# THUDM/GCC

Measured on NVIDIA H100. Metric: subgraphs/sec (MoCo pretrain step), higher is better.
Workload: dtype f32

## Files before the change

gcc_b200/csrc/sampler.cu:

```cuda
#include "common.cuh"

namespace gccb {

__global__ void draw_seeds_kernel(const double* __restrict__ cdf, int64_t n, uint64_t key,
                                  int64_t first, int count, int64_t* __restrict__ seeds,
                                  int64_t* __restrict__ sample_ids) {
  int i = blockIdx.x * blockDim.x + threadIdx.x;
  if (i >= count) return;
  uint64_t sample = (uint64_t)(first + i);
  u32x4 w = philox_at(key, sample, 0, 0, 0, GCCB_TAG_SEED);
  uint64_t u53 = ((uint64_t)w.x << 21) | (uint64_t)(w.y >> 11);
  double u = (double)u53 * (1.0 / 9007199254740992.0);
  int64_t lo = 0, hi = n;
  while (lo < hi) {
    int64_t mid = (lo + hi) >> 1;
    if (cdf[mid] > u) hi = mid; else lo = mid + 1;
  }
  seeds[i] = lo < n ? lo : n - 1;
  if (sample_ids) sample_ids[i] = first + i;
}

__device__ __forceinline__ int local_id(const int* keys, int n, int seed, int u) {
  if (u == seed) return 0;
  int lo = 1, hi = n;
// ... 3 lines not shown
  }
  return (lo < n && keys[lo] == u) ? lo : -1;
}

__device__ __forceinline__ unsigned bloom_bit(int u) { return ((unsigned)u * 2654435761u) >> 16; }

__device__ __forceinline__ int adj_count(const int32_t* __restrict__ indices, int64_t beg, int64_t end, int u) {
  const int64_t stop = end;
  while (beg < end) {
    int64_t mid = (beg + end) >> 1;
    if (indices[mid] < u) beg = mid + 1; else end = mid;
  }
  if (beg >= stop || indices[beg] != u) return 0;
  const int32_t* run = indices + beg;
  int lo = 1, hi = (int)min(stop - beg, (int64_t)0x7fffffff);
  if (lo == hi || run[lo] != u) return 1;
  while (lo < hi) {
    int mid = (lo + hi) >> 1;
    if (run[mid] <= u) lo = mid + 1; else hi = mid;
  }
  return lo;
}
#define GCCB_REVERSE_FACTOR 16
#ifndef GCCB_ST
#define GCCB_ST 1024
#endif
#define GCCB_SW (GCCB_ST / 32)
#ifndef GCCB_SCAN_UNROLL
#define GCCB_SCAN_UNROLL 4
#endif
#ifndef GCCB_BLOOM
#define GCCB_BLOOM 1
#endif
#define GCCB_BLOOM_WORDS 2048
#ifndef GCCB_HUB_LIST
#define GCCB_HUB_LIST 1024
#endif
#define GCCB_HIT_STAGE 128
#ifndef GCCB_WALK_KEYS
#define GCCB_WALK_KEYS 32768
#endif
#define GCCB_WALK_BUDGET_MAX (GCCB_WALK_KEYS - (int)GCCB_HOPCAP)
#define GCCB_WIDE_CTAS 32
#define GCCB_WIDE_KEYS_MAX (1 << 30)

__device__ void block_sort_pad(int* a, int cnt) {
  const int tid = threadIdx.x;
  int P = 1;
  while (P < cnt) P <<= 1;
  for (int i = cnt + tid; i < P; i += GCCB_ST) a[i] = 0x7fffffff;
  __syncthreads();
  for (int k = 2; k <= P; k <<= 1) {
    for (int j = k >> 1; j > 0; j >>= 1) {
      for (int i = tid; i < P; i += GCCB_ST) {
        const int ixj = i ^ j;
        if (ixj > i) {
          const int x = a[i], y = a[ixj];
          if ((x > y) == ((i & k) == 0)) { a[i] = y; a[ixj] = x; }
        }
      }
      __syncthreads();
    }
  }
}

__device__ __forceinline__ bool in_sorted(const int* a, int n, int u) {
  int lo = 0, hi = n;
  while (lo < hi) { const int mid = (lo + hi) >> 1; if (a[mid] < u) lo = mid + 1; else hi = mid; }
  return lo < n && a[lo] == u;
}

__device__ int ns_expand(const int64_t* __restrict__ indptr, const int32_t* __restrict__ indices, uint64_t key,
                         uint64_t sample, uint32_t view, int seed, int hops, int k, int cap, int* V, int* F, int* S,
                         int* scan_scratch, int32_t* __restrict__ subv, int* layers) {
  __shared__ int s_miss;
  const int tid = threadIdx.x, lane = tid & 31, warp = tid >> 5;
  int nV = 1, nF = 1, checked = 0, hop = 1;
// ... 7 lines not shown
      int64_t beg = 0, d = 0;
      if (i < nF) { beg = indptr[F[i]]; d = indptr[F[i] + 1] - beg; }
      int tot;
      const int ex = block_scan_excl(d <= k ? (int)d : k, scan_scratch, &tot);
      if (i < nF) {
        int* out = S + nc + ex;
        if (d <= k) {
          for (int e = 0; e < (int)d; ++e) out[e] = indices[beg + e];
        } else {
          for (int t = 0; t < k; ++t) {
            const uint32_t j = (uint32_t)(d - k + t);
            const u32x4 w = philox_at(key, sample, (uint32_t)i | ((uint32_t)t << 16), c3hop, view, c3tag);
            const int r = (int)__umulhi(w.x, j + 1u);
            bool dup = false;
            for (int q = 0; q < t; ++q) dup |= out[q] == r;
            out[t] = dup ? (int)j : r;
          }
          for (int t = 0; t < k; ++t) out[t] = indices[beg + out[t]];
        }
      }
      nc += tot;
    }
    __syncthreads();
    block_sort_pad(S, nc);
    int nF2 = 0;
    for (int b0 = 0; b0 < nc; b0 += GCCB_ST) {
      const int i = b0 + tid;
      const int head = i < nc && (i == 0 || S[i - 1] != S[i]);
      int tot;
      const int ex = block_scan_excl(head, scan_scratch, &tot);
      if (head && nF2 + ex < cap) F[nF2 + ex] = S[i];
      nF2 += tot;
    }
    if (nF2 > cap) return -1;
    nF = nF2;
    __syncthreads();
    if (nF == 0) break;
    int nNew = 0;
    for (int b0 = 0; b0 < nF; b0 += GCCB_ST) {
      const int i = b0 + tid;
      const int fresh = i < nF && !in_sorted(V, nV, F[i]);
      int tot;
      const int ex = block_scan_excl(fresh, scan_scratch, &tot);
      if (fresh) S[nV + nNew + ex] = F[i];
      nNew += tot;
    }
    if (nV + nNew > cap) return -1;
    if (nNew > 0) {
      for (int i = tid; i < nV; i += GCCB_ST) S[i] = V[i];
      block_sort_pad(S, nV + nNew);
      nV += nNew;
      for (int i = tid; i < nV; i += GCCB_ST) V[i] = S[i];
      __syncthreads();
    } else if (nV != checked) {
      if (tid == 0) s_miss = 0;
      __syncthreads();
      int miss = 0;
      for (int i = warp; i < nV; i += GCCB_SW) {
        const int64_t end = indptr[V[i] + 1];
        for (int64_t e = indptr[V[i]] + lane; e < end && !miss; e += 32) miss = !in_sorted(V, nV, indices[e]);
      }
      if (miss) s_miss = 1;
      __syncthreads();
      const bool closed = s_miss == 0;
      __syncthreads();
      if (closed) break;
      checked = nV;
    }
  }
  *layers = hop > hops ? hops : hop;
  for (int i = tid; i < nV; i += GCCB_ST) {
    const int v = V[i];
    subv[v < seed ? i + 1 : (v == seed ? 0 : i)] = v;
  }
  return nV;
}

__device__ __forceinline__ int rwr_node_set(const int64_t* __restrict__ indptr, const int32_t* __restrict__ indices,
                                            int budget, uint32_t restart_thresh, uint64_t key, uint64_t sample,
                                            int view, int64_t seed64, int seed, int* keys, int* scan_scratch,
                                            int* s_tstar, int* s_m, int32_t* __restrict__ flags,
                                            int32_t* rest, int* steps) {
  const int tid = threadIdx.x;
  if (tid == 0) *s_tstar = 0x7fffffff;
  __syncthreads();

  int base = 0;
  int total = 0;
  for (int chunk = 0;; ++chunk) {
    const uint32_t t = (uint32_t)(chunk * GCCB_ST + tid);
    int len = 1;
    for (uint32_t hop = 1; hop < GCCB_HOPCAP; ++hop) {
      u32x4 w = philox_at(key, sample, t, hop, (uint32_t)view, GCCB_TAG_WALK);
      if (w.x < restart_thresh) break;
      ++len;
    }
    int chunk_total;
    int excl = block_scan_excl(len, scan_scratch, &chunk_total);
    int cum = base + excl + len;
    if (cum >= budget && cum - len < budget) *s_tstar = (int)t;
    __syncthreads();
    const int tstar = *s_tstar;
    if ((int)t <= tstar) {
      int64_t cur = seed64;
      int pos = base + excl;
      for (uint32_t hop = 0; hop < (uint32_t)len; ++hop) {
        u32x4 w = philox_at(key, sample, t, hop, (uint32_t)view, GCCB_TAG_WALK);
        int64_t beg = indptr[cur];
        uint32_t deg = (uint32_t)(indptr[cur + 1] - beg);
        if (deg == 0u) { atomicOr(flags, (int)GCCB_FLAG_ZERO_DEGREE); keys[pos++] = (int)cur; continue; }
        cur = indices[beg + __umulhi(w.y, deg)];
        keys[pos++] = (int)cur;
      }
    }
    if (tstar != 0x7fffffff) {
      if ((int)t == tstar) *s_m = cum;
      __syncthreads();
      total = *s_m;
      break;
    }
    base += chunk_total;
    __syncthreads();
  }
  __syncthreads();
  if (tid == 0) *s_m = 0;

  int P = 1;
  while (P < total) P <<= 1;
  for (int i = total + tid; i < P; i += GCCB_ST) keys[i] = 0x7fffffff;
  __syncthreads();
  for (int k = 2; k <= P; k <<= 1) {
    for (int j = k >> 1; j > 0; j >>= 1) {
      for (int i = tid; i < P; i += GCCB_ST) {
        int ixj = i ^ j;
        if (ixj > i) {
          int a = keys[i], b = keys[ixj];
          bool asc = (i & k) == 0;
          if ((a > b) == asc) { keys[i] = b; keys[ixj] = a; }
        }
      }
      __syncthreads();
    }
  }
  int n_rest = 0;
  for (int b0 = 0; b0 < total; b0 += GCCB_ST) {
    int i = b0 + tid;
    int head = 0, v = 0;
    if (i < total) {
      v = keys[i];
      head = (v != seed) && (i == 0 || keys[i - 1] != v);
    }
    int cnt;
    int ex = block_scan_excl(head, scan_scratch, &cnt);
    if (head) rest[n_rest + ex] = v;
    n_rest += cnt;
  }
  *steps = total;
  return n_rest + 1;
}

enum { kModeRwr = 0, kModePairs = 1, kModeNs = 2 };

struct WideWs {
  int32_t* subv;
  int32_t* subdeg;
  int32_t* rowstart;
  unsigned long long* used;
  unsigned* next;
  int region;
};

template <int kMode, bool kWide>
__device__ __forceinline__ void
walk_slot(const int slot, int* keys, const int64_t* __restrict__ indptr, const int32_t* __restrict__ indices,
          int64_t n_nodes, const int32_t* __restrict__ budget_table, int budget_table_len, uint32_t restart_thresh,
          uint64_t key, const int64_t* __restrict__ seeds, const int64_t* __restrict__ sample_ids, int B, int cap_n,
          int32_t* __restrict__ subv_scratch, int32_t* __restrict__ subdeg_scratch,
          int32_t* __restrict__ rowstart_scratch, int32_t* __restrict__ pool, int pool_cap,
          unsigned long long* __restrict__ pool_counter, int64_t* __restrict__ counters,
          int32_t* __restrict__ flags, const int64_t* __restrict__ seeds_k, int ns_hops, int ns_k, int node_cap,
          const WideWs& wide) {
  __shared__ int scan_scratch[33];
  __shared__ int stage[GCCB_SW][GCCB_HIT_STAGE];
  __shared__ int s_tstar, s_m;
  __shared__ unsigned long long s_sumdeg;
  __shared__ int s_nhub, s_pos;
  __shared__ unsigned bloom[GCCB_BLOOM_WORDS];
  __shared__ int hub_rows[GCCB_HUB_LIST];
  const int tid = threadIdx.x, lane = tid & 31, warp = tid >> 5;
  const int view = slot / B, g = slot - view * B;
  int64_t seed64 = seeds[g];
  seed64 = seed64 < 0 ? 0 : (seed64 >= n_nodes ? n_nodes - 1 : seed64);
  const int64_t q64 = seed64;
  if constexpr (kMode != kModeRwr) {
    if (view == 1) {
      seed64 = seeds_k[g];
      seed64 = seed64 < 0 ? 0 : (seed64 >= n_nodes ? n_nodes - 1 : seed64);
    }
  }
  const int seed = (int)seed64;
  const uint64_t sample = (uint64_t)sample_ids[g];
  int32_t* subv = subv_scratch + (size_t)slot * cap_n;
  int32_t* subdeg = subdeg_scratch + (size_t)slot * cap_n;
  int32_t* rowstart = rowstart_scratch + (size_t)slot * cap_n;
  if (tid == 0) { s_m = 0; s_sumdeg = 0ull; }
  int n, total = 0;
  if constexpr (kMode == kModeNs) {
    n = ns_expand(indptr, indices, key, sample, (uint32_t)view, seed, ns_hops, ns_k, cap_n, keys, keys + cap_n,
                  keys + 2 * cap_n, scan_scratch, subv, &total);
    if (n < 0) {
      if (tid == 0) {
        counters[(size_t)slot * 4 + 0] = (int64_t)node_cap + 1;
        counters[(size_t)slot * 4 + 1] = 0;
        counters[(size_t)slot * 4 + 2] = total;
        counters[(size_t)slot * 4 + 3] = 0;
        atomicOr(flags, (int)GCCB_FLAG_NODE_OVERFLOW);
      }
      return;
    }
    __syncthreads();
  } else {
    const int64_t sdeg = indptr[q64 + 1] - indptr[q64];
    const int budget = budget_table[sdeg < budget_table_len ? (int)sdeg : budget_table_len - 1];
    if constexpr (!kWide) {
      if (budget > GCCB_WALK_BUDGET_MAX) {
        if (tid == 0) subv[0] = -1;
        return;
      }
    }
    n = rwr_node_set(indptr, indices, budget, restart_thresh, key, sample, view, seed64, seed, keys, scan_scratch,
                     &s_tstar, &s_m, flags, kWide ? keys : subv + 1, &total);
  }
  if constexpr (kWide) {
    if (tid == 0) {
      const unsigned long long off = atomicAdd(wide.used + view, (unsigned long long)n);
      s_pos = off + (unsigned long long)n <= (unsigned long long)wide.region ? (int)off : -1;
      subv[1] = s_pos;
    }
    __syncthreads();
    const int off = s_pos;
    if (off < 0) {
      if (tid == 0) {
        counters[(size_t)slot * 4 + 0] = n;
        counters[(size_t)slot * 4 + 1] = n - 1;
        counters[(size_t)slot * 4 + 2] = total;
        counters[(size_t)slot * 4 + 3] = 0;
      }
      return;
    }
    const size_t at = (size_t)view * wide.region + off;
    subv = wide.subv + at;
    subdeg = wide.subdeg + at;
    rowstart = wide.rowstart + at;
    for (int i = tid; i < n - 1; i += GCCB_ST) subv[1 + i] = keys[i];
    if (tid == 0) subv[0] = seed;
    keys = subv;
  } else {
    if (tid == 0) subv[0] = seed;
    __syncthreads();
    for (int i = tid; i < n; i += GCCB_ST) keys[i] = subv[i];
  }
  for (int i = tid; i < GCCB_BLOOM_WORDS; i += GCCB_ST) bloom[i] = 0u;
  __syncthreads();
  for (int i = tid; i < n; i += GCCB_ST) {
    const unsigned b = bloom_bit(keys[i]);
    atomicOr(&bloom[b >> 5], 1u << (b & 31u));
  }
  __syncthreads();

  int* wstage = stage[warp];
  const unsigned lt_mask = (1u << lane) - 1u;
  int m_local = 0;
  unsigned long long sumdeg_local = 0ull;
  int sr = 0;
  {
    int lo = 1, hi = n;
    while (lo < hi) { int mid = (lo + hi) >> 1; if (keys[mid] < seed) lo = mid + 1; else hi = mid; }
    sr = lo - 1;
  }
  if (tid == 0) s_nhub = 0;
  __syncthreads();
  for (int i = tid; i < n; i += GCCB_ST) {
    const int64_t v = keys[i];
    int mark = -3;
    if (indptr[v + 1] - indptr[v] > (int64_t)GCCB_REVERSE_FACTOR * n) {
      const int idx = atomicAdd(&s_nhub, 1);
      if (idx < GCCB_HUB_LIST) { hub_rows[idx] = i; mark = -2; }
    }
    rowstart[i] = mark;
  }
  __syncthreads();
  const int n_hub = min(s_nhub, GCCB_HUB_LIST);
  for (int h = 0; h < n_hub; ++h) {
    const int i = hub_rows[h];
    const int64_t v = keys[i];
    const int64_t beg = indptr[v], end = indptr[v + 1];
    int cnt = 0, my_j = 0, my_c = 0, my_ex = 0;
    for (int t0 = 0; t0 < n; t0 += GCCB_ST) {
      const int t = t0 + tid;
      int j = 0, c = 0;
      if (t < n) {
        j = t < sr ? t + 1 : (t == sr ? 0 : t);
        c = adj_count(indices, beg, end, keys[j]);
      }
      int tot;
      const int ex = block_scan_excl(c, scan_scratch, &tot);
      if (t0 == 0) { my_j = j; my_c = c; my_ex = ex; }
      cnt += tot;
    }
    if (tid == 0) {
      const unsigned long long p64 = cnt > 0 ? atomicAdd(pool_counter, (unsigned long long)cnt) : 0ull;
      s_pos = p64 + (unsigned long long)cnt > (unsigned long long)pool_cap ? -1 : (int)p64;
    }
    __syncthreads();
    const int pos = s_pos;
    if (pos >= 0) {
      if (n <= GCCB_ST) {
        for (int k = 0; k < my_c; ++k) pool[pos + my_ex + k] = my_j;
      } else {
        int w = 0;
        for (int t0 = 0; t0 < n; t0 += GCCB_ST) {
          const int t = t0 + tid;
          int j = 0, c = 0;
          if (t < n) {
            j = t < sr ? t + 1 : (t == sr ? 0 : t);
            c = adj_count(indices, beg, end, keys[j]);
          }
          int tot;
          const int ex = block_scan_excl(c, scan_scratch, &tot);
          for (int k = 0; k < c; ++k) pool[pos + w + ex + k] = j;
          w += tot;
        }
      }
    }
    if (tid == 0) {
      subdeg[i] = cnt;
      rowstart[i] = pos;
      m_local += cnt;
      sumdeg_local += (unsigned long long)(end - beg);
    }
    __syncthreads();
  }
  for (int i = warp; i < n; i += GCCB_SW) {
    if (rowstart[i] != -3) continue;
    const int64_t v = keys[i];
    const int64_t beg = indptr[v], end = indptr[v + 1];
    const bool reverse = end - beg > (int64_t)GCCB_REVERSE_FACTOR * n;
    int pos = 0, w = 0, round = 0;
    auto emit = [&](int j) {
      const unsigned hit = __ballot_sync(0xffffffffu, j >= 0);
      if (j >= 0) {
        const int q = w + __popc(hit & lt_mask);
        if (round == 1) pool[pos + q] = j;
        else if (q < GCCB_HIT_STAGE) wstage[q] = j;
      }
      w += __popc(hit);
    };
    auto scan_row = [&]() {
      w = 0;
      if (reverse) {
        for (int t0 = 0; t0 < n; t0 += 32) {
          const int t = t0 + lane;
          int j = 0, c = 0;
          if (t < n) {
            j = t < sr ? t + 1 : (t == sr ? 0 : t);
            c = adj_count(indices, beg, end, keys[j]);
// ... 47 lines not shown
    }
    __syncwarp();
    if (lane == 0) {
      subdeg[i] = cnt;
      rowstart[i] = pos;
      m_local += cnt;
      sumdeg_local += (unsigned long long)(end - beg);
    }
  }
  if (lane == 0) {
    atomicAdd(&s_m, m_local);
    atomicAdd(&s_sumdeg, sumdeg_local);
  }
  __syncthreads();
  if (tid == 0) {
    counters[(size_t)slot * 4 + 0] = n;
    counters[(size_t)slot * 4 + 1] = s_m;
    counters[(size_t)slot * 4 + 2] = total;
    counters[(size_t)slot * 4 + 3] = (int64_t)s_sumdeg;
  }
}

template <int kMode>
__global__ void __launch_bounds__(GCCB_ST)
rwr_walk_unique_kernel(const int64_t* __restrict__ indptr, const int32_t* __restrict__ indices, int64_t n_nodes,
                       const int32_t* __restrict__ budget_table, int budget_table_len,
                       uint32_t restart_thresh, uint64_t key, const int64_t* __restrict__ seeds,
                       const int64_t* __restrict__ sample_ids, int B, int cap_n,
                       int32_t* __restrict__ subv_scratch, int32_t* __restrict__ subdeg_scratch,
                       int32_t* __restrict__ rowstart_scratch, int32_t* __restrict__ pool, int pool_cap,
                       unsigned long long* __restrict__ pool_counter,
                       int64_t* __restrict__ counters, int32_t* __restrict__ flags,
                       const int64_t* __restrict__ seeds_k, int ns_hops, int ns_k, int node_cap) {
  GCCB_DYN_SMEM(int, keys);
  walk_slot<kMode, false>(blockIdx.x, keys, indptr, indices, n_nodes, budget_table, budget_table_len, restart_thresh,
                          key, seeds, sample_ids, B, cap_n, subv_scratch, subdeg_scratch, rowstart_scratch, pool,
                          pool_cap, pool_counter, counters, flags, seeds_k, ns_hops, ns_k, node_cap, WideWs{});
}

template <int kMode>
__global__ void __launch_bounds__(GCCB_ST)
rwr_walk_wide_kernel(const int64_t* __restrict__ indptr, const int32_t* __restrict__ indices, int64_t n_nodes,
                     const int32_t* __restrict__ budget_table, int budget_table_len,
                     uint32_t restart_thresh, uint64_t key, const int64_t* __restrict__ seeds,
                     const int64_t* __restrict__ sample_ids, int B, int cap_n,
                     int32_t* __restrict__ subv_scratch, int32_t* __restrict__ pool, int pool_cap,
                     unsigned long long* __restrict__ pool_counter,
                     int64_t* __restrict__ counters, int32_t* __restrict__ flags,
                     const int64_t* __restrict__ seeds_k, WideWs wide, int32_t* __restrict__ wide_keys,
                     size_t keys_len) {
  __shared__ int s_slot;
  int* keys = wide_keys + (size_t)blockIdx.x * keys_len;
  for (;;) {
    if (threadIdx.x == 0) s_slot = (int)atomicAdd(wide.next, 1u);
    __syncthreads();
    const int slot = s_slot;
    if (slot >= 2 * B) return;
    if (subv_scratch[(size_t)slot * cap_n] < 0)
      walk_slot<kMode, true>(slot, keys, indptr, indices, n_nodes, budget_table, budget_table_len, restart_thresh,
                             key, seeds, sample_ids, B, cap_n, subv_scratch, nullptr, nullptr, pool, pool_cap,
                             pool_counter, counters, flags, seeds_k, 0, 0, 0, wide);
    __syncthreads();
  }
}

__global__ void __launch_bounds__(256)
batch_offsets_kernel(const int64_t* __restrict__ counters, int B, int node_cap, int edge_cap,
                     int32_t* __restrict__ node_off, int32_t* __restrict__ edge_off,
                     int32_t* __restrict__ flags) {
  __shared__ int scan_scratch[33];
  const int view = blockIdx.x, tid = threadIdx.x;
  long long nbase = 0, ebase = 0;
  for (int b0 = 0; b0 < B; b0 += 256) {
    int g = b0 + tid;
    int n = 0, m = 0;
    if (g < B) {
      n = (int)counters[(size_t)(view * B + g) * 4 + 0];
      m = (int)counters[(size_t)(view * B + g) * 4 + 1];
    }
    int tn, tm;
    int en = block_scan_excl(n, scan_scratch, &tn);
    int em = block_scan_excl(m, scan_scratch, &tm);
    if (g < B) {
      long long no = nbase + en, eo = ebase + em;
      node_off[view * (B + 1) + g] = (int)(no > 0x7fffffffLL ? 0x7fffffffLL : no);
      edge_off[view * (B + 1) + g] = (int)(eo > 0x7fffffffLL ? 0x7fffffffLL : eo);
    }
    nbase += tn;
    ebase += tm;
  }
  if (tid == 0) {
    int f = 0;
    if (nbase > node_cap) { f |= GCCB_FLAG_NODE_OVERFLOW; }
    if (ebase > edge_cap) { f |= GCCB_FLAG_EDGE_OVERFLOW; }
    node_off[view * (B + 1) + B] = f ? -1 : (int)nbase;
    edge_off[view * (B + 1) + B] = f ? -1 : (int)ebase;
    if (f) atomicOr(flags, f);
  }
}

template <bool kWide>
__device__ __forceinline__ void
fill_slot(const int slot, int* keys, const int64_t* __restrict__ indptr, const int32_t* __restrict__ indices,
          const int64_t* __restrict__ counters, int B, int node_cap, int edge_cap, const int32_t* __restrict__ subv,
          const int32_t* __restrict__ subdeg, const int32_t* __restrict__ rowstart, const int32_t* __restrict__ pool,
          int32_t* __restrict__ node_off, const int32_t* __restrict__ edge_off, int32_t* __restrict__ out_indptr,
          int32_t* __restrict__ out_indices, int32_t* __restrict__ out_subdeg, int32_t* __restrict__ out_graph_id,
          int32_t* __restrict__ out_orig_id) {
  __shared__ int scan_scratch[33];
  const int tid = threadIdx.x, lane = tid & 31, warp = tid >> 5;
  const int view = slot / B, g = slot - view * B;
  const int Nv = node_off[view * (B + 1) + B];
  if (Nv < 0) return;
  const int n = (int)counters[(size_t)slot * 4 + 0];
  const int noff = node_off[view * (B + 1) + g];
  const int eoff = edge_off[view * (B + 1) + g];
  int32_t* v_indptr = out_indptr + (size_t)view * (node_cap + 1);
  int32_t* v_indices = out_indices + (size_t)view * edge_cap;
  const size_t nb = (size_t)view * node_cap;
  if constexpr (!kWide)
    for (int i = tid; i < n; i += GCCB_ST) keys[i] = subv[i];
  const int seed = subv[0];
  int run = 0;
  for (int b0 = 0; b0 < n; b0 += GCCB_ST) {
    int i = b0 + tid;
    int d = i < n ? subdeg[i] : 0;
    int tot;
    int ex = block_scan_excl(d, scan_scratch, &tot);
    if (i < n) {
      v_indptr[noff + i] = eoff + run + ex;
      out_subdeg[nb + noff + i] = d;
      out_graph_id[nb + noff + i] = g;
      out_orig_id[nb + noff + i] = subv[i];
    }
    run += tot;
  }
  if (g == B - 1 && tid == 0) v_indptr[noff + n] = eoff + run;
  __syncthreads();
  for (int i = warp; i < n; i += GCCB_SW) {
    int wpos = v_indptr[noff + i];
    const int rs = rowstart[i];
    if (rs >= 0) {
      const int d = subdeg[i];
      for (int q = lane; q < d; q += 32) v_indices[wpos + q] = noff + pool[rs + q];
      continue;
    }
    const int64_t v = keys[i];
    const int64_t beg = indptr[v], end = indptr[v + 1];
    if (end - beg > (int64_t)GCCB_REVERSE_FACTOR * n) {
      int lo = 1, hi = n;
      while (lo < hi) { int mid = (lo + hi) >> 1; if (keys[mid] < seed) lo = mid + 1; else hi = mid; }
      const int sr = lo - 1;
      for (int t0 = 0; t0 < n; t0 += 32) {
        const int t = t0 + lane;
        int j = 0, c = 0;
        if (t < n) {
          j = t < sr ? t + 1 : (t == sr ? 0 : t);
          c = adj_count(indices, beg, end, keys[j]);
        }
        const int incl = warp_scan_incl(c, lane);
        for (int q = wpos + incl - c; q < wpos + incl; ++q) v_indices[q] = noff + j;
        wpos += __shfl_sync(0xffffffffu, incl, 31);
      }
      continue;
    }
    for (int64_t e0 = beg; e0 < end; e0 += 32) {
      int64_t e = e0 + lane;
      int j = -1;
      if (e < end) j = local_id(keys, n, seed, indices[e]);
      unsigned hit = __ballot_sync(0xffffffffu, j >= 0);
      if (j >= 0) v_indices[wpos + __popc(hit & ((1u << lane) - 1u))] = noff + j;
      wpos += __popc(hit);
    }
  }
}

__global__ void __launch_bounds__(GCCB_ST)
induce_fill_kernel(const int64_t* __restrict__ indptr, const int32_t* __restrict__ indices,
                   const int64_t* __restrict__ counters, int B, int cap_n, int node_cap,
                   int edge_cap, const int32_t* __restrict__ subv_scratch,
                   const int32_t* __restrict__ subdeg_scratch, const int32_t* __restrict__ rowstart_scratch,
                   const int32_t* __restrict__ pool,
                   int32_t* __restrict__ node_off, const int32_t* __restrict__ edge_off,
                   int32_t* __restrict__ out_indptr, int32_t* __restrict__ out_indices,
                   int32_t* __restrict__ out_subdeg, int32_t* __restrict__ out_graph_id,
                   int32_t* __restrict__ out_orig_id) {
  GCCB_DYN_SMEM(int, keys);
  const int slot = blockIdx.x;
  const size_t at = (size_t)slot * cap_n;
  if (subv_scratch[at] < 0) return;
  fill_slot<false>(slot, keys, indptr, indices, counters, B, node_cap, edge_cap, subv_scratch + at,
                   subdeg_scratch + at, rowstart_scratch + at, pool, node_off, edge_off, out_indptr, out_indices,
                   out_subdeg, out_graph_id, out_orig_id);
}

__global__ void __launch_bounds__(GCCB_ST)
induce_fill_wide_kernel(const int64_t* __restrict__ indptr, const int32_t* __restrict__ indices,
                        const int64_t* __restrict__ counters, int B, int cap_n, int node_cap, int edge_cap,
                        const int32_t* __restrict__ subv_scratch, WideWs wide, const int32_t* __restrict__ pool,
                        int32_t* __restrict__ node_off, const int32_t* __restrict__ edge_off,
                        int32_t* __restrict__ out_indptr, int32_t* __restrict__ out_indices,
                        int32_t* __restrict__ out_subdeg, int32_t* __restrict__ out_graph_id,
                        int32_t* __restrict__ out_orig_id) {
  const int slot = blockIdx.x;
  const int32_t* mark = subv_scratch + (size_t)slot * cap_n;
  if (mark[0] >= 0 || mark[1] < 0) return;
  const size_t at = (size_t)(slot / B) * wide.region + mark[1];
  fill_slot<true>(slot, wide.subv + at, indptr, indices, counters, B, node_cap, edge_cap, wide.subv + at,
                  wide.subdeg + at, wide.rowstart + at, pool, node_off, edge_off, out_indptr, out_indices,
                  out_subdeg, out_graph_id, out_orig_id);
}

__global__ void pair_seeds_kernel(const int64_t* __restrict__ indptr, const int32_t* __restrict__ indices,
                                  int64_t n_nodes, uint64_t key, double cdf0, double cdf1, int n_steps,
                                  const int64_t* __restrict__ seeds_q, const int64_t* __restrict__ sample_ids,
                                  int count, int64_t* __restrict__ seeds_k) {
  const int i = blockIdx.x * blockDim.x + threadIdx.x;
  if (i >= count) return;
  const uint64_t sample = (uint64_t)sample_ids[i];
  const u32x4 w = philox_at(key, sample, 0, 0, 0, GCCB_TAG_STEP);
  const double u = (double)(((uint64_t)w.x << 21) | (uint64_t)(w.y >> 11)) * (1.0 / 9007199254740992.0);
  int step = 0;
  if (step < n_steps - 1 && !(cdf0 > u)) ++step;
  if (step == 1 && step < n_steps - 1 && !(cdf1 > u)) ++step;
  int64_t cur = seeds_q[i];
  cur = cur < 0 ? 0 : (cur >= n_nodes ? n_nodes - 1 : cur);
  for (int h = 1; h <= step; ++h) {
    const int64_t beg = indptr[cur];
    const uint32_t deg = (uint32_t)(indptr[cur + 1] - beg);
    if (deg == 0u) break;
    const u32x4 r = philox_at(key, sample, 0, (uint32_t)h, 0, GCCB_TAG_KHOP);
// ... 8 lines not shown

static int pow2_ge(int x) { int p = 1; while (p < x) p <<= 1; return p; }

extern "C" int gccb_draw_seeds(const double* cdf, int64_t n_nodes, uint64_t key,
                               int64_t first_sample, int32_t count, int64_t* seeds_out,
                               int64_t* sample_ids_out, gccb_stream_t stream) {
  if (!cdf || !seeds_out || n_nodes <= 0 || count < 0) {
    set_last_error("gccb_draw_seeds: bad argument");
    return GCCB_ERR_BADARG;
  }
  if (count == 0) return GCCB_OK;
  GCCB_LAUNCH(draw_seeds_kernel, (count + 127) / 128, 128, 0, stream, cdf, n_nodes, key,
              first_sample, count, seeds_out, sample_ids_out);
  return check_launch("draw_seeds_kernel");
}

static int sampler_cap_n(int max_budget) { return (max_budget + (int)GCCB_HOPCAP + 1 + 3) & ~3; }
static bool sampler_wide(int max_budget) { return max_budget > GCCB_WALK_BUDGET_MAX; }
static int wide_region(int batch, int edge_cap) {
  const long long r = (long long)edge_cap + batch;
  return (int)(r < 0x7fffffffll ? r : 0x7fffffffll);
}
static int wide_ctas(int batch) { return 2 * batch < GCCB_WIDE_CTAS ? 2 * batch : GCCB_WIDE_CTAS; }
static size_t wide_keys_len(int max_budget) {
  size_t p = 1;
  while (p < (size_t)max_budget + GCCB_HOPCAP) p <<= 1;
  return p;
}

extern "C" size_t gccb_sample_batch_workspace(int32_t batch, int32_t max_budget, int32_t edge_cap) {
  const bool wide = sampler_wide(max_budget);
  const int cap_n = sampler_cap_n(wide ? GCCB_WALK_BUDGET_MAX : max_budget);
  size_t ints = (size_t)3 * (size_t)(2 * batch) * (size_t)cap_n + 16 + (size_t)2 * (size_t)edge_cap;
  if (wide)
    ints += (size_t)6 * (size_t)wide_region(batch, edge_cap) + (size_t)wide_ctas(batch) * wide_keys_len(max_budget);
  return ints * sizeof(int32_t);
}

template <int kMode>
static int sample_batch_rwr(const char* what, const gccb_graph_t* graph, const int64_t* seeds, const int64_t* seeds_k,
                            const int64_t* sample_ids, const gccb_batch_t* batch, void* workspace,
                            size_t workspace_bytes, gccb_stream_t stream) {
  const int B = batch->batch;
  const bool wide = sampler_wide(graph->max_budget);
  if (wide && wide_keys_len(graph->max_budget) > (size_t)GCCB_WIDE_KEYS_MAX) {
    set_last_error("%s: walk budget %d: a trace of up to %d vertices does not fit int32 positions", what,
                   graph->max_budget, graph->max_budget + (int)GCCB_HOPCAP - 1);
    return GCCB_ERR_CAPACITY;
  }
  const int cap_n = sampler_cap_n(wide ? GCCB_WALK_BUDGET_MAX : graph->max_budget);
  if (workspace_bytes < gccb_sample_batch_workspace(B, graph->max_budget, batch->edge_cap)) {
    set_last_error("%s: workspace too small", what);
    return GCCB_ERR_CAPACITY;
  }
  const int P = wide ? GCCB_WALK_KEYS : pow2_ge(graph->max_budget + (int)GCCB_HOPCAP);
  const size_t smem = (size_t)P * sizeof(int);
  int32_t* subv = (int32_t*)workspace;
  int32_t* subdeg = subv + (size_t)2 * B * cap_n;
  int32_t* rowstart = subdeg + (size_t)2 * B * cap_n;
  unsigned long long* pool_counter = (unsigned long long*)(rowstart + (size_t)2 * B * cap_n);
  int32_t* pool = (int32_t*)pool_counter + 16;
  const long long want_cap = 2ll * (long long)batch->edge_cap;
  const int pool_cap = (int)(want_cap < 0x7fff0000ll ? want_cap : 0x7fff0000ll);
  cudaMemsetAsync(pool_counter, 0, wide ? 16 * sizeof(int32_t) : sizeof(unsigned long long), (cudaStream_t)stream);
  auto k1 = rwr_walk_unique_kernel<kMode>;
  auto k3 = induce_fill_kernel;
  if (smem > 48 * 1024) {
    gccb::ensure_dyn_smem(k1, smem);
    gccb::ensure_dyn_smem(k3, smem);
  }
  GCCB_LAUNCH(k1, 2 * B, GCCB_ST, smem, stream, graph->indptr, graph->indices, graph->n_nodes, graph->budget_table,
              graph->budget_table_len, graph->restart_thresh, graph->key, seeds, sample_ids, B,
              cap_n, subv, subdeg, rowstart, pool, pool_cap, pool_counter, batch->counters, batch->flags,
              seeds_k, 0, 0, 0);
  WideWs ww = {};
  if (wide) {
    ww.region = wide_region(B, batch->edge_cap);
    ww.subv = pool + (size_t)2 * batch->edge_cap;
    ww.subdeg = ww.subv + (size_t)2 * ww.region;
    ww.rowstart = ww.subdeg + (size_t)2 * ww.region;
    ww.used = pool_counter + 2;
    ww.next = (unsigned*)(pool_counter + 1);
    int32_t* wide_keys = ww.rowstart + (size_t)2 * ww.region;
    GCCB_LAUNCH(rwr_walk_wide_kernel<kMode>, wide_ctas(B), GCCB_ST, 0, stream, graph->indptr, graph->indices,
                graph->n_nodes, graph->budget_table, graph->budget_table_len, graph->restart_thresh, graph->key,
                seeds, sample_ids, B, cap_n, subv, pool, pool_cap, pool_counter, batch->counters, batch->flags,
                seeds_k, ww, wide_keys, wide_keys_len(graph->max_budget));
  }
  GCCB_LAUNCH(batch_offsets_kernel, 2, 256, 0, stream, batch->counters, B, batch->node_cap,
              batch->edge_cap, batch->node_off, batch->edge_off, batch->flags);
  GCCB_LAUNCH(k3, 2 * B, GCCB_ST, smem, stream, graph->indptr, graph->indices, batch->counters, B,
              cap_n, batch->node_cap, batch->edge_cap, subv, subdeg, rowstart, pool, batch->node_off,
              batch->edge_off, batch->indptr, batch->indices, batch->sub_deg, batch->graph_id,
              batch->orig_id);
  if (wide)
    GCCB_LAUNCH(induce_fill_wide_kernel, 2 * B, GCCB_ST, 0, stream, graph->indptr, graph->indices, batch->counters,
                B, cap_n, batch->node_cap, batch->edge_cap, subv, ww, pool, batch->node_off, batch->edge_off,
                batch->indptr, batch->indices, batch->sub_deg, batch->graph_id, batch->orig_id);
  return check_launch(what);
}

extern "C" int gccb_sample_batch(const gccb_graph_t* graph, const int64_t* seeds,
                                 const int64_t* sample_ids, const gccb_batch_t* batch,
                                 void* workspace, size_t workspace_bytes, gccb_stream_t stream) {
  if (!graph || !batch || !seeds || !sample_ids || !workspace || batch->batch <= 0 ||
      graph->max_budget <= 0 || !graph->indptr || !graph->indices || !graph->budget_table) {
    set_last_error("gccb_sample_batch: bad argument");
    return GCCB_ERR_BADARG;
  }
  return sample_batch_rwr<kModeRwr>("gccb_sample_batch", graph, seeds, (const int64_t*)nullptr, sample_ids, batch,
                                    workspace, workspace_bytes, stream);
}


extern "C" int gccb_pair_seeds(const gccb_graph_t* graph, const double* step_cdf, int32_t n_steps,
                               const int64_t* seeds_q, const int64_t* sample_ids, int32_t count, int64_t* seeds_k,
                               gccb_stream_t stream) {
// ... 46 lines not shown
      !graph->indptr || !graph->indices || graph->n_nodes <= 0 || num_hops < 0 || num_hops > 0xffff || cap == 0) {
    set_last_error("gccb_ns_batch: bad argument (num_hops 0..65535, num_neighbors 1..%d)", 0xffff);
    return GCCB_ERR_BADARG;
  }
  if (batch->node_cap > GCCB_NS_NODE_CAP_MAX) {
    set_last_error("gccb_ns_batch: node_cap %d above %d", batch->node_cap, GCCB_NS_NODE_CAP_MAX);
    return GCCB_ERR_CAPACITY;
  }
  const int B = batch->batch;
  if (workspace_bytes < gccb_ns_batch_workspace(B, num_neighbors, batch->edge_cap)) {
    set_last_error("gccb_ns_batch: workspace too small");
    return GCCB_ERR_CAPACITY;
  }
  const size_t smem1 = ns_smem(cap, num_neighbors), smem3 = (size_t)cap * sizeof(int);
  int32_t* subv = (int32_t*)workspace;
  int32_t* subdeg = subv + (size_t)2 * B * cap;
  int32_t* rowstart = subdeg + (size_t)2 * B * cap;
  unsigned long long* pool_counter = (unsigned long long*)(rowstart + (size_t)2 * B * cap);
  int32_t* pool = (int32_t*)pool_counter + 16;
  const long long want_cap = 2ll * (long long)batch->edge_cap;
  const int pool_cap = (int)(want_cap < 0x7fff0000ll ? want_cap : 0x7fff0000ll);
  cudaMemsetAsync(pool_counter, 0, sizeof(unsigned long long), (cudaStream_t)stream);
  auto k1 = rwr_walk_unique_kernel<kModeNs>;
  auto k3 = induce_fill_kernel;
  if (smem1 > 48 * 1024) gccb::ensure_dyn_smem(k1, smem1);
  if (smem3 > 48 * 1024) gccb::ensure_dyn_smem(k3, smem3);
  GCCB_LAUNCH(k1, 2 * B, GCCB_ST, smem1, stream, graph->indptr, graph->indices, graph->n_nodes,
              (const int32_t*)nullptr, 0, 0u, graph->key, seeds_q, sample_ids, B, cap, subv, subdeg, rowstart, pool,
              pool_cap, pool_counter, batch->counters, batch->flags, seeds_k, (int)num_hops, (int)num_neighbors,
              batch->node_cap);
  GCCB_LAUNCH(batch_offsets_kernel, 2, 256, 0, stream, batch->counters, B, batch->node_cap,
              batch->edge_cap, batch->node_off, batch->edge_off, batch->flags);
  GCCB_LAUNCH(k3, 2 * B, GCCB_ST, smem3, stream, graph->indptr, graph->indices, batch->counters, B,
              cap, batch->node_cap, batch->edge_cap, subv, subdeg, rowstart, pool, batch->node_off,
              batch->edge_off, batch->indptr, batch->indices, batch->sub_deg, batch->graph_id,
              batch->orig_id);
  return check_launch("gccb_ns_batch");
}
```

Measured before the change: 255,900.

## Split RWR sampling into small-CTA ordinary tier and side-stream hub tier

Seeds are classified by walk budget into three tiers. Ordinary seeds run in 256-thread CTAs with 4 KB of keys, which allows several CTAs per SM. Hub seeds go to a persistent kernel with a few 1024-thread CTAs on a side stream, forked and joined with events so it overlaps the ordinary work. The wide path is unchanged apart from an explicit marker value. The aim is to stop the largest budget from fixing the shared-memory and thread size of every CTA, at the cost of extra launches, recomputing the tier in the fill kernel, and cross-stream synchronisation.

New measurement: 261,600, median of 6. 1.02x the previous value.

```diff
diff --git a/gcc_b200/csrc/sampler.cu b/gcc_b200/csrc/sampler.cu
--- a/gcc_b200/csrc/sampler.cu
+++ b/gcc_b200/csrc/sampler.cu
@@ -49,10 +49,13 @@
   return lo;
 }
 #define GCCB_REVERSE_FACTOR 16
-#ifndef GCCB_ST
 #define GCCB_ST 1024
+#define GCCB_ORD_ST 256
+#ifndef GCCB_ORD_KEYS
+#define GCCB_ORD_KEYS 1024
 #endif
-#define GCCB_SW (GCCB_ST / 32)
+#define GCCB_ORD_BUDGET_MAX (GCCB_ORD_KEYS - (int)GCCB_HOPCAP)
+#define GCCB_HUB_CTAS 8
 #ifndef GCCB_SCAN_UNROLL
 #define GCCB_SCAN_UNROLL 4
 #endif
@@ -70,16 +73,18 @@
 #define GCCB_WALK_BUDGET_MAX (GCCB_WALK_KEYS - (int)GCCB_HOPCAP)
 #define GCCB_WIDE_CTAS 32
 #define GCCB_WIDE_KEYS_MAX (1 << 30)
-
+static_assert(GCCB_ORD_KEYS <= GCCB_WALK_KEYS, "the ordinary tier's budgets lie below the hub tier's");
+
+template <int NT>
 __device__ void block_sort_pad(int* a, int cnt) {
   const int tid = threadIdx.x;
   int P = 1;
   while (P < cnt) P <<= 1;
-  for (int i = cnt + tid; i < P; i += GCCB_ST) a[i] = 0x7fffffff;
+  for (int i = cnt + tid; i < P; i += NT) a[i] = 0x7fffffff;
   __syncthreads();
   for (int k = 2; k <= P; k <<= 1) {
     for (int j = k >> 1; j > 0; j >>= 1) {
-      for (int i = tid; i < P; i += GCCB_ST) {
+      for (int i = tid; i < P; i += NT) {
         const int ixj = i ^ j;
         if (ixj > i) {
           const int x = a[i], y = a[ixj];
@@ -133,7 +138,7 @@
       nc += tot;
     }
     __syncthreads();
-    block_sort_pad(S, nc);
+    block_sort_pad<GCCB_ST>(S, nc);
     int nF2 = 0;
     for (int b0 = 0; b0 < nc; b0 += GCCB_ST) {
       const int i = b0 + tid;
@@ -159,7 +164,7 @@
     if (nV + nNew > cap) return -1;
     if (nNew > 0) {
       for (int i = tid; i < nV; i += GCCB_ST) S[i] = V[i];
-      block_sort_pad(S, nV + nNew);
+      block_sort_pad<GCCB_ST>(S, nV + nNew);
       nV += nNew;
       for (int i = tid; i < nV; i += GCCB_ST) V[i] = S[i];
       __syncthreads();
@@ -167,7 +172,7 @@
       if (tid == 0) s_miss = 0;
       __syncthreads();
       int miss = 0;
-      for (int i = warp; i < nV; i += GCCB_SW) {
+      for (int i = warp; i < nV; i += GCCB_ST / 32) {
         const int64_t end = indptr[V[i] + 1];
         for (int64_t e = indptr[V[i]] + lane; e < end && !miss; e += 32) miss = !in_sorted(V, nV, indices[e]);
       }
@@ -187,6 +192,7 @@
   return nV;
 }
 
+template <int NT>
 __device__ __forceinline__ int rwr_node_set(const int64_t* __restrict__ indptr, const int32_t* __restrict__ indices,
                                             int budget, uint32_t restart_thresh, uint64_t key, uint64_t sample,
                                             int view, int64_t seed64, int seed, int* keys, int* scan_scratch,
@@ -199,7 +205,7 @@
   int base = 0;
   int total = 0;
   for (int chunk = 0;; ++chunk) {
-    const uint32_t t = (uint32_t)(chunk * GCCB_ST + tid);
+    const uint32_t t = (uint32_t)(chunk * NT + tid);
     int len = 1;
     for (uint32_t hop = 1; hop < GCCB_HOPCAP; ++hop) {
       u32x4 w = philox_at(key, sample, t, hop, (uint32_t)view, GCCB_TAG_WALK);
@@ -236,25 +242,9 @@
   __syncthreads();
   if (tid == 0) *s_m = 0;
 
-  int P = 1;
-  while (P < total) P <<= 1;
-  for (int i = total + tid; i < P; i += GCCB_ST) keys[i] = 0x7fffffff;
-  __syncthreads();
-  for (int k = 2; k <= P; k <<= 1) {
-    for (int j = k >> 1; j > 0; j >>= 1) {
-      for (int i = tid; i < P; i += GCCB_ST) {
-        int ixj = i ^ j;
-        if (ixj > i) {
-          int a = keys[i], b = keys[ixj];
-          bool asc = (i & k) == 0;
-          if ((a > b) == asc) { keys[i] = b; keys[ixj] = a; }
-        }
-      }
-      __syncthreads();
-    }
-  }
+  block_sort_pad<NT>(keys, total);
   int n_rest = 0;
-  for (int b0 = 0; b0 < total; b0 += GCCB_ST) {
+  for (int b0 = 0; b0 < total; b0 += NT) {
     int i = b0 + tid;
     int head = 0, v = 0;
     if (i < total) {
@@ -281,7 +271,20 @@
   int region;
 };
 
-template <int kMode, bool kWide>
+enum { kTierOrd = 0, kTierHub = 1, kTierWide = 2 };
+enum { kMarkWide = -1 };
+
+__device__ __forceinline__ int budget_tier(int budget) {
+  return budget <= GCCB_ORD_BUDGET_MAX ? kTierOrd : (budget <= GCCB_WALK_BUDGET_MAX ? kTierHub : kTierWide);
+}
+
+__device__ __forceinline__ int walk_budget(const int64_t* __restrict__ indptr, const int32_t* __restrict__ budget_table,
+                                           int budget_table_len, int64_t q64) {
+  const int64_t sdeg = indptr[q64 + 1] - indptr[q64];
+  return budget_table[sdeg < budget_table_len ? (int)sdeg : budget_table_len - 1];
+}
+
+template <int kMode, int kTier, int NT>
 __device__ __forceinline__ void
 walk_slot(const int slot, int* keys, const int64_t* __restrict__ indptr, const int32_t* __restrict__ indices,
           int64_t n_nodes, const int32_t* __restrict__ budget_table, int budget_table_len, uint32_t restart_thresh,
@@ -291,8 +294,9 @@
           unsigned long long* __restrict__ pool_counter, int64_t* __restrict__ counters,
           int32_t* __restrict__ flags, const int64_t* __restrict__ seeds_k, int ns_hops, int ns_k, int node_cap,
           const WideWs& wide) {
+  constexpr bool kWide = kTier == kTierWide;
   __shared__ int scan_scratch[33];
-  __shared__ int stage[GCCB_SW][GCCB_HIT_STAGE];
+  __shared__ int stage[NT / 32][GCCB_HIT_STAGE];
   __shared__ int s_tstar, s_m;
   __shared__ unsigned long long s_sumdeg;
   __shared__ int s_nhub, s_pos;
@@ -331,15 +335,15 @@
     }
     __syncthreads();
   } else {
-    const int64_t sdeg = indptr[q64 + 1] - indptr[q64];
-    const int budget = budget_table[sdeg < budget_table_len ? (int)sdeg : budget_table_len - 1];
-    if constexpr (!kWide) {
-      if (budget > GCCB_WALK_BUDGET_MAX) {
-        if (tid == 0) subv[0] = -1;
+    const int budget = walk_budget(indptr, budget_table, budget_table_len, q64);
+    if constexpr (kTier == kTierOrd) {
+      const int tier = budget_tier(budget);
+      if (tier != kTierOrd) {
+        if (tid == 0 && tier == kTierWide) subv[0] = kMarkWide;
         return;
       }
     }
-    n = rwr_node_set(indptr, indices, budget, restart_thresh, key, sample, view, seed64, seed, keys, scan_scratch,
+    n = rwr_node_set<NT>(indptr, indices, budget, restart_thresh, key, sample, view, seed64, seed, keys, scan_scratch,
                      &s_tstar, &s_m, flags, kWide ? keys : subv + 1, &total);
   }
   if constexpr (kWide) {
@@ -363,17 +367,17 @@
     subv = wide.subv + at;
     subdeg = wide.subdeg + at;
     rowstart = wide.rowstart + at;
-    for (int i = tid; i < n - 1; i += GCCB_ST) subv[1 + i] = keys[i];
+    for (int i = tid; i < n - 1; i += NT) subv[1 + i] = keys[i];
     if (tid == 0) subv[0] = seed;
     keys = subv;
   } else {
     if (tid == 0) subv[0] = seed;
     __syncthreads();
-    for (int i = tid; i < n; i += GCCB_ST) keys[i] = subv[i];
-  }
-  for (int i = tid; i < GCCB_BLOOM_WORDS; i += GCCB_ST) bloom[i] = 0u;
+    for (int i = tid; i < n; i += NT) keys[i] = subv[i];
+  }
+  for (int i = tid; i < GCCB_BLOOM_WORDS; i += NT) bloom[i] = 0u;
   __syncthreads();
-  for (int i = tid; i < n; i += GCCB_ST) {
+  for (int i = tid; i < n; i += NT) {
     const unsigned b = bloom_bit(keys[i]);
     atomicOr(&bloom[b >> 5], 1u << (b & 31u));
   }
@@ -391,7 +395,7 @@
   }
   if (tid == 0) s_nhub = 0;
   __syncthreads();
-  for (int i = tid; i < n; i += GCCB_ST) {
+  for (int i = tid; i < n; i += NT) {
     const int64_t v = keys[i];
     int mark = -3;
     if (indptr[v + 1] - indptr[v] > (int64_t)GCCB_REVERSE_FACTOR * n) {
@@ -407,7 +411,7 @@
     const int64_t v = keys[i];
     const int64_t beg = indptr[v], end = indptr[v + 1];
     int cnt = 0, my_j = 0, my_c = 0, my_ex = 0;
-    for (int t0 = 0; t0 < n; t0 += GCCB_ST) {
+    for (int t0 = 0; t0 < n; t0 += NT) {
       const int t = t0 + tid;
       int j = 0, c = 0;
       if (t < n) {
@@ -426,11 +430,11 @@
     __syncthreads();
     const int pos = s_pos;
     if (pos >= 0) {
-      if (n <= GCCB_ST) {
+      if (n <= NT) {
         for (int k = 0; k < my_c; ++k) pool[pos + my_ex + k] = my_j;
       } else {
         int w = 0;
-        for (int t0 = 0; t0 < n; t0 += GCCB_ST) {
+        for (int t0 = 0; t0 < n; t0 += NT) {
           const int t = t0 + tid;
           int j = 0, c = 0;
           if (t < n) {
@@ -452,7 +456,7 @@
     }
     __syncthreads();
   }
-  for (int i = warp; i < n; i += GCCB_SW) {
+  for (int i = warp; i < n; i += NT / 32) {
     if (rowstart[i] != -3) continue;
     const int64_t v = keys[i];
     const int64_t beg = indptr[v], end = indptr[v + 1];
@@ -546,7 +550,7 @@
 }
 
 template <int kMode>
-__global__ void __launch_bounds__(GCCB_ST)
+__global__ void __launch_bounds__(kMode == kModeNs ? GCCB_ST : GCCB_ORD_ST, kMode == kModeNs ? 1 : 4)
 rwr_walk_unique_kernel(const int64_t* __restrict__ indptr, const int32_t* __restrict__ indices, int64_t n_nodes,
                        const int32_t* __restrict__ budget_table, int budget_table_len,
                        uint32_t restart_thresh, uint64_t key, const int64_t* __restrict__ seeds,
@@ -557,9 +561,65 @@
                        int64_t* __restrict__ counters, int32_t* __restrict__ flags,
                        const int64_t* __restrict__ seeds_k, int ns_hops, int ns_k, int node_cap) {
   GCCB_DYN_SMEM(int, keys);
-  walk_slot<kMode, false>(blockIdx.x, keys, indptr, indices, n_nodes, budget_table, budget_table_len, restart_thresh,
-                          key, seeds, sample_ids, B, cap_n, subv_scratch, subdeg_scratch, rowstart_scratch, pool,
-                          pool_cap, pool_counter, counters, flags, seeds_k, ns_hops, ns_k, node_cap, WideWs{});
+  if constexpr (kMode == kModeNs) {
+    walk_slot<kMode, kTierOrd, GCCB_ST>(blockIdx.x, keys, indptr, indices, n_nodes, budget_table, budget_table_len,
+                                        restart_thresh, key, seeds, sample_ids, B, cap_n, subv_scratch, subdeg_scratch,
+                                        rowstart_scratch, pool, pool_cap, pool_counter, counters, flags, seeds_k,
+                                        ns_hops, ns_k, node_cap, WideWs{});
+  } else {
+    walk_slot<kMode, kTierOrd, GCCB_ORD_ST>(blockIdx.x, keys, indptr, indices, n_nodes, budget_table,
+                                            budget_table_len, restart_thresh, key, seeds, sample_ids, B, cap_n,
+                                            subv_scratch, subdeg_scratch, rowstart_scratch, pool, pool_cap,
+                                            pool_counter, counters, flags, seeds_k, 0, 0, 0, WideWs{});
+  }
+}
+
+template <class F>
+__device__ __forceinline__ void for_each_hub_slot(const int64_t* __restrict__ indptr, int64_t n_nodes,
+                                                  const int32_t* __restrict__ budget_table, int budget_table_len,
+                                                  const int64_t* __restrict__ seeds, int B, F&& visit) {
+  __shared__ int scan_scratch[33];
+  __shared__ int list[GCCB_ST];
+  const int G = gridDim.x;
+  int before = 0;
+  for (int b0 = 0; b0 < 2 * B; b0 += GCCB_ST) {
+    const int slot = b0 + threadIdx.x;
+    int hub = 0;
+    if (slot < 2 * B) {
+      int64_t q64 = seeds[slot % B];
+      q64 = q64 < 0 ? 0 : (q64 >= n_nodes ? n_nodes - 1 : q64);
+      hub = budget_tier(walk_budget(indptr, budget_table, budget_table_len, q64)) == kTierHub;
+    }
+    int tot;
+    const int ex = block_scan_excl(hub, scan_scratch, &tot);
+    if (hub) list[ex] = slot;
+    __syncthreads();
+    for (int j = (int)((blockIdx.x + (unsigned)G - (unsigned)(before % G)) % (unsigned)G); j < tot; j += G) {
+      visit(list[j]);
+      __syncthreads();
+    }
+    before += tot;
+  }
+}
+
+template <int kMode>
+__global__ void __launch_bounds__(GCCB_ST)
+rwr_walk_hub_kernel(const int64_t* __restrict__ indptr, const int32_t* __restrict__ indices, int64_t n_nodes,
+                    const int32_t* __restrict__ budget_table, int budget_table_len,
+                    uint32_t restart_thresh, uint64_t key, const int64_t* __restrict__ seeds,
+                    const int64_t* __restrict__ sample_ids, int B, int cap_n,
+                    int32_t* __restrict__ subv_scratch, int32_t* __restrict__ subdeg_scratch,
+                    int32_t* __restrict__ rowstart_scratch, int32_t* __restrict__ pool, int pool_cap,
+                    unsigned long long* __restrict__ pool_counter,
+                    int64_t* __restrict__ counters, int32_t* __restrict__ flags,
+                    const int64_t* __restrict__ seeds_k) {
+  GCCB_DYN_SMEM(int, keys);
+  for_each_hub_slot(indptr, n_nodes, budget_table, budget_table_len, seeds, B, [&](int slot) {
+    walk_slot<kMode, kTierHub, GCCB_ST>(slot, keys, indptr, indices, n_nodes, budget_table, budget_table_len,
+                                        restart_thresh, key, seeds, sample_ids, B, cap_n, subv_scratch, subdeg_scratch,
+                                        rowstart_scratch, pool, pool_cap, pool_counter, counters, flags, seeds_k, 0, 0,
+                                        0, WideWs{});
+  });
 }
 
 template <int kMode>
@@ -580,10 +640,11 @@
     __syncthreads();
     const int slot = s_slot;
     if (slot >= 2 * B) return;
-    if (subv_scratch[(size_t)slot * cap_n] < 0)
-      walk_slot<kMode, true>(slot, keys, indptr, indices, n_nodes, budget_table, budget_table_len, restart_thresh,
-                             key, seeds, sample_ids, B, cap_n, subv_scratch, nullptr, nullptr, pool, pool_cap,
-                             pool_counter, counters, flags, seeds_k, 0, 0, 0, wide);
+    if (subv_scratch[(size_t)slot * cap_n] == kMarkWide)
+      walk_slot<kMode, kTierWide, GCCB_ST>(slot, keys, indptr, indices, n_nodes, budget_table, budget_table_len,
+                                           restart_thresh, key, seeds, sample_ids, B, cap_n, subv_scratch, nullptr,
+                                           nullptr, pool, pool_cap, pool_counter, counters, flags, seeds_k, 0, 0, 0,
+                                           wide);
     __syncthreads();
   }
 }
@@ -623,7 +684,7 @@
   }
 }
 
-template <bool kWide>
+template <bool kWide, int NT>
 __device__ __forceinline__ void
 fill_slot(const int slot, int* keys, const int64_t* __restrict__ indptr, const int32_t* __restrict__ indices,
           const int64_t* __restrict__ counters, int B, int node_cap, int edge_cap, const int32_t* __restrict__ subv,
@@ -643,10 +704,10 @@
   int32_t* v_indices = out_indices + (size_t)view * edge_cap;
   const size_t nb = (size_t)view * node_cap;
   if constexpr (!kWide)
-    for (int i = tid; i < n; i += GCCB_ST) keys[i] = subv[i];
+    for (int i = tid; i < n; i += NT) keys[i] = subv[i];
   const int seed = subv[0];
   int run = 0;
-  for (int b0 = 0; b0 < n; b0 += GCCB_ST) {
+  for (int b0 = 0; b0 < n; b0 += NT) {
     int i = b0 + tid;
     int d = i < n ? subdeg[i] : 0;
     int tot;
@@ -661,7 +722,7 @@
   }
   if (g == B - 1 && tid == 0) v_indptr[noff + n] = eoff + run;
   __syncthreads();
-  for (int i = warp; i < n; i += GCCB_SW) {
+  for (int i = warp; i < n; i += NT / 32) {
     int wpos = v_indptr[noff + i];
     const int rs = rowstart[i];
     if (rs >= 0) {
@@ -699,8 +760,9 @@
   }
 }
 
-__global__ void __launch_bounds__(GCCB_ST)
-induce_fill_kernel(const int64_t* __restrict__ indptr, const int32_t* __restrict__ indices,
+__global__ void __launch_bounds__(GCCB_ORD_ST, 4)
+induce_fill_kernel(const int64_t* __restrict__ indptr, const int32_t* __restrict__ indices, int64_t n_nodes,
+                   const int32_t* __restrict__ budget_table, int budget_table_len, const int64_t* __restrict__ seeds,
                    const int64_t* __restrict__ counters, int B, int cap_n, int node_cap,
                    int edge_cap, const int32_t* __restrict__ subv_scratch,
                    const int32_t* __restrict__ subdeg_scratch, const int32_t* __restrict__ rowstart_scratch,
@@ -711,11 +773,49 @@
                    int32_t* __restrict__ out_orig_id) {
   GCCB_DYN_SMEM(int, keys);
   const int slot = blockIdx.x;
+  int64_t q64 = seeds[slot % B];
+  q64 = q64 < 0 ? 0 : (q64 >= n_nodes ? n_nodes - 1 : q64);
+  if (budget_tier(walk_budget(indptr, budget_table, budget_table_len, q64)) != kTierOrd) return;
   const size_t at = (size_t)slot * cap_n;
-  if (subv_scratch[at] < 0) return;
-  fill_slot<false>(slot, keys, indptr, indices, counters, B, node_cap, edge_cap, subv_scratch + at,
-                   subdeg_scratch + at, rowstart_scratch + at, pool, node_off, edge_off, out_indptr, out_indices,
-                   out_subdeg, out_graph_id, out_orig_id);
+  fill_slot<false, GCCB_ORD_ST>(slot, keys, indptr, indices, counters, B, node_cap, edge_cap, subv_scratch + at,
+                                subdeg_scratch + at, rowstart_scratch + at, pool, node_off, edge_off, out_indptr,
+                                out_indices, out_subdeg, out_graph_id, out_orig_id);
+}
+
+__global__ void __launch_bounds__(GCCB_ST)
+induce_fill_ns_kernel(const int64_t* __restrict__ indptr, const int32_t* __restrict__ indices,
+                      const int64_t* __restrict__ counters, int B, int cap_n, int node_cap,
+                      int edge_cap, const int32_t* __restrict__ subv_scratch,
+                      const int32_t* __restrict__ subdeg_scratch, const int32_t* __restrict__ rowstart_scratch,
+                      const int32_t* __restrict__ pool,
+                      int32_t* __restrict__ node_off, const int32_t* __restrict__ edge_off,
+                      int32_t* __restrict__ out_indptr, int32_t* __restrict__ out_indices,
+                      int32_t* __restrict__ out_subdeg, int32_t* __restrict__ out_graph_id,
+                      int32_t* __restrict__ out_orig_id) {
+  GCCB_DYN_SMEM(int, keys);
+  const size_t at = (size_t)blockIdx.x * cap_n;
+  fill_slot<false, GCCB_ST>(blockIdx.x, keys, indptr, indices, counters, B, node_cap, edge_cap, subv_scratch + at,
+                            subdeg_scratch + at, rowstart_scratch + at, pool, node_off, edge_off, out_indptr,
+                            out_indices, out_subdeg, out_graph_id, out_orig_id);
+}
+
+__global__ void __launch_bounds__(GCCB_ST)
+induce_fill_hub_kernel(const int64_t* __restrict__ indptr, const int32_t* __restrict__ indices, int64_t n_nodes,
+                       const int32_t* __restrict__ budget_table, int budget_table_len,
+                       const int64_t* __restrict__ seeds, const int64_t* __restrict__ counters, int B, int cap_n,
+                       int node_cap, int edge_cap, const int32_t* __restrict__ subv_scratch,
+                       const int32_t* __restrict__ subdeg_scratch, const int32_t* __restrict__ rowstart_scratch,
+                       const int32_t* __restrict__ pool, int32_t* __restrict__ node_off,
+                       const int32_t* __restrict__ edge_off, int32_t* __restrict__ out_indptr,
+                       int32_t* __restrict__ out_indices, int32_t* __restrict__ out_subdeg,
+                       int32_t* __restrict__ out_graph_id, int32_t* __restrict__ out_orig_id) {
+  GCCB_DYN_SMEM(int, keys);
+  for_each_hub_slot(indptr, n_nodes, budget_table, budget_table_len, seeds, B, [&](int slot) {
+    const size_t at = (size_t)slot * cap_n;
+    fill_slot<false, GCCB_ST>(slot, keys, indptr, indices, counters, B, node_cap, edge_cap, subv_scratch + at,
+                              subdeg_scratch + at, rowstart_scratch + at, pool, node_off, edge_off, out_indptr,
+                              out_indices, out_subdeg, out_graph_id, out_orig_id);
+  });
 }
 
 __global__ void __launch_bounds__(GCCB_ST)
@@ -728,9 +828,9 @@
                         int32_t* __restrict__ out_orig_id) {
   const int slot = blockIdx.x;
   const int32_t* mark = subv_scratch + (size_t)slot * cap_n;
-  if (mark[0] >= 0 || mark[1] < 0) return;
+  if (mark[0] != kMarkWide || mark[1] < 0) return;
   const size_t at = (size_t)(slot / B) * wide.region + mark[1];
-  fill_slot<true>(slot, wide.subv + at, indptr, indices, counters, B, node_cap, edge_cap, wide.subv + at,
+  fill_slot<true, GCCB_ST>(slot, wide.subv + at, indptr, indices, counters, B, node_cap, edge_cap, wide.subv + at,
                   wide.subdeg + at, wide.rowstart + at, pool, node_off, edge_off, out_indptr, out_indices,
                   out_subdeg, out_graph_id, out_orig_id);
 }
@@ -785,6 +885,17 @@
   return (int)(r < 0x7fffffffll ? r : 0x7fffffffll);
 }
 static int wide_ctas(int batch) { return 2 * batch < GCCB_WIDE_CTAS ? 2 * batch : GCCB_WIDE_CTAS; }
+static int hub_ctas(int batch) { return 2 * batch < GCCB_HUB_CTAS ? 2 * batch : GCCB_HUB_CTAS; }
+
+template <class K>
+static void fit_dyn_smem(K kern, size_t dyn) {
+  size_t stat = 0;
+#ifndef GCCB_EMU
+  cudaFuncAttributes a;
+  if (cudaFuncGetAttributes(&a, kern) == cudaSuccess) stat = a.sharedSizeBytes;
+#endif
+  if (stat + dyn > 48 * 1024) gccb::ensure_dyn_smem(kern, dyn);
+}
 static size_t wide_keys_len(int max_budget) {
   size_t p = 1;
   while (p < (size_t)max_budget + GCCB_HOPCAP) p <<= 1;
@@ -816,8 +927,8 @@
     set_last_error("%s: workspace too small", what);
     return GCCB_ERR_CAPACITY;
   }
-  const int P = wide ? GCCB_WALK_KEYS : pow2_ge(graph->max_budget + (int)GCCB_HOPCAP);
-  const size_t smem = (size_t)P * sizeof(int);
+  const bool hub = graph->max_budget > GCCB_ORD_BUDGET_MAX;
+  const size_t hub_smem = (size_t)(wide ? GCCB_WALK_KEYS : pow2_ge(graph->max_budget + (int)GCCB_HOPCAP)) * sizeof(int);
   int32_t* subv = (int32_t*)workspace;
   int32_t* subdeg = subv + (size_t)2 * B * cap_n;
   int32_t* rowstart = subdeg + (size_t)2 * B * cap_n;
@@ -826,16 +937,39 @@
   const long long want_cap = 2ll * (long long)batch->edge_cap;
   const int pool_cap = (int)(want_cap < 0x7fff0000ll ? want_cap : 0x7fff0000ll);
   cudaMemsetAsync(pool_counter, 0, wide ? 16 * sizeof(int32_t) : sizeof(unsigned long long), (cudaStream_t)stream);
-  auto k1 = rwr_walk_unique_kernel<kMode>;
-  auto k3 = induce_fill_kernel;
-  if (smem > 48 * 1024) {
-    gccb::ensure_dyn_smem(k1, smem);
-    gccb::ensure_dyn_smem(k3, smem);
-  }
-  GCCB_LAUNCH(k1, 2 * B, GCCB_ST, smem, stream, graph->indptr, graph->indices, graph->n_nodes, graph->budget_table,
-              graph->budget_table_len, graph->restart_thresh, graph->key, seeds, sample_ids, B,
-              cap_n, subv, subdeg, rowstart, pool, pool_cap, pool_counter, batch->counters, batch->flags,
-              seeds_k, 0, 0, 0);
+  gccb_stream_t hub_stream = stream;
+#ifndef GCCB_EMU
+  cudaEvent_t* ev = nullptr;
+  if (hub) {
+    StreamKit* kit = stream_kit((cudaStream_t)stream, 3);
+    hub_stream = kit->side[0];
+    ev = kit->ev;
+  }
+  auto fork = [&](int e) {
+    cudaEventRecord(ev[e], (cudaStream_t)stream);
+    cudaStreamWaitEvent((cudaStream_t)hub_stream, ev[e], 0);
+  };
+  auto join = [&](int e) {
+    cudaEventRecord(ev[e], (cudaStream_t)hub_stream);
+    cudaStreamWaitEvent((cudaStream_t)stream, ev[e], 0);
+  };
+#else
+  auto fork = [](int) {};
+  auto join = [](int) {};
+#endif
+  if (hub) {
+    fork(0);
+    fit_dyn_smem(rwr_walk_hub_kernel<kMode>, hub_smem);
+    GCCB_LAUNCH(rwr_walk_hub_kernel<kMode>, hub_ctas(B), GCCB_ST, hub_smem, hub_stream, graph->indptr, graph->indices,
+                graph->n_nodes, graph->budget_table, graph->budget_table_len, graph->restart_thresh, graph->key,
+                seeds, sample_ids, B, cap_n, subv, subdeg, rowstart, pool, pool_cap, pool_counter, batch->counters,
+                batch->flags, seeds_k);
+  }
+  GCCB_LAUNCH(rwr_walk_unique_kernel<kMode>, 2 * B, GCCB_ORD_ST, GCCB_ORD_KEYS * sizeof(int), stream, graph->indptr, graph->indices,
+              graph->n_nodes, graph->budget_table, graph->budget_table_len, graph->restart_thresh, graph->key, seeds,
+              sample_ids, B, cap_n, subv, subdeg, rowstart, pool, pool_cap, pool_counter, batch->counters,
+              batch->flags, seeds_k, 0, 0, 0);
+  if (hub) join(1);
   WideWs ww = {};
   if (wide) {
     ww.region = wide_region(B, batch->edge_cap);
@@ -852,10 +986,19 @@
   }
   GCCB_LAUNCH(batch_offsets_kernel, 2, 256, 0, stream, batch->counters, B, batch->node_cap,
               batch->edge_cap, batch->node_off, batch->edge_off, batch->flags);
-  GCCB_LAUNCH(k3, 2 * B, GCCB_ST, smem, stream, graph->indptr, graph->indices, batch->counters, B,
+  if (hub) {
+    fork(2);
+    fit_dyn_smem(induce_fill_hub_kernel, hub_smem);
+    GCCB_LAUNCH(induce_fill_hub_kernel, hub_ctas(B), GCCB_ST, hub_smem, hub_stream, graph->indptr, graph->indices,
+                graph->n_nodes, graph->budget_table, graph->budget_table_len, seeds, batch->counters, B, cap_n,
+                batch->node_cap, batch->edge_cap, subv, subdeg, rowstart, pool, batch->node_off, batch->edge_off,
+                batch->indptr, batch->indices, batch->sub_deg, batch->graph_id, batch->orig_id);
+  }
+  GCCB_LAUNCH(induce_fill_kernel, 2 * B, GCCB_ORD_ST, GCCB_ORD_KEYS * sizeof(int), stream, graph->indptr,
+              graph->indices, graph->n_nodes, graph->budget_table, graph->budget_table_len, seeds, batch->counters, B,
               cap_n, batch->node_cap, batch->edge_cap, subv, subdeg, rowstart, pool, batch->node_off,
-              batch->edge_off, batch->indptr, batch->indices, batch->sub_deg, batch->graph_id,
-              batch->orig_id);
+              batch->edge_off, batch->indptr, batch->indices, batch->sub_deg, batch->graph_id, batch->orig_id);
+  if (hub) join(3);
   if (wide)
     GCCB_LAUNCH(induce_fill_wide_kernel, 2 * B, GCCB_ST, 0, stream, graph->indptr, graph->indices, batch->counters,
                 B, cap_n, batch->node_cap, batch->edge_cap, subv, ww, pool, batch->node_off, batch->edge_off,
@@ -948,9 +1091,9 @@
   const int pool_cap = (int)(want_cap < 0x7fff0000ll ? want_cap : 0x7fff0000ll);
   cudaMemsetAsync(pool_counter, 0, sizeof(unsigned long long), (cudaStream_t)stream);
   auto k1 = rwr_walk_unique_kernel<kModeNs>;
-  auto k3 = induce_fill_kernel;
-  if (smem1 > 48 * 1024) gccb::ensure_dyn_smem(k1, smem1);
-  if (smem3 > 48 * 1024) gccb::ensure_dyn_smem(k3, smem3);
+  auto k3 = induce_fill_ns_kernel;
+  fit_dyn_smem(k1, smem1);
+  fit_dyn_smem(k3, smem3);
   GCCB_LAUNCH(k1, 2 * B, GCCB_ST, smem1, stream, graph->indptr, graph->indices, graph->n_nodes,
               (const int32_t*)nullptr, 0, 0u, graph->key, seeds_q, sample_ids, B, cap, subv, subdeg, rowstart, pool,
               pool_cap, pool_counter, batch->counters, batch->flags, seeds_k, (int)num_hops, (int)num_neighbors,
```
